# Aakash1312/Fluid-Simulation

Measured on AMD Instinct MI355X. Metric: simulated substeps/sec, higher is better.
Workload: dtype f64

## Files before the change

fluid-simulation_amd/_lib.py:

```python
import ctypes as C
import os

_HERE = os.path.dirname(os.path.abspath(__file__))
_SO = os.path.join(_HERE, "libfluid_hip.so")
if not os.path.exists(_SO):
    raise ImportError(
        f"{_SO} is missing: build it with `make -C {_HERE}` (hipcc --offload-arch=gfx950). "
        "This package has no CPU path.")
lib = C.CDLL(_SO)


class FluidError(RuntimeError):
    def __init__(self, code, msg):
        super().__init__(f"libfluid_hip error {code}: {msg}")
        self.code = code


class Params(C.Structure):
    _fields_ = [("n", C.c_int32), ("device", C.c_int32), ("dx", C.c_double), ("rho", C.c_double),
                ("gravity", C.c_double * 3), ("max_dt", C.c_double), ("outer_tol", C.c_double),
                ("update_frac", C.c_double), ("cg_tol", C.c_double), ("cg_max_iters", C.c_int32),
                ("max_outer_passes", C.c_int32), ("precision", C.c_int32), ("preconditioner", C.c_int32),
                ("flip_blend", C.c_double), ("solve_start", C.c_int32), ("mg_precision", C.c_int32),
                ("dist_solve", C.c_int32), ("pad_", C.c_int32)]
# ... 116 lines not shown
SYMBOLS = [
    ("fluid_default_params", C.c_int, [C.POINTER(Params)]),
    ("fluid_create", C.c_int, [C.POINTER(Params), C.POINTER(_P)]),
    ("fluid_destroy", C.c_int, [_P]),
    ("fluid_last_error", C.c_char_p, []),
    ("fluid_version", C.c_char_p, []),
    ("fluid_set_solid", C.c_int, [_P, _P]),
    ("fluid_upload_particles", C.c_int, [_P, C.c_int64, _P, _P]),
    ("fluid_download_particles", C.c_int, [_P, _P, _P]),
    ("fluid_num_particles", C.c_int64, [_P]),
    ("fluid_set_dt", C.c_int, [_P, C.c_double]),
    ("fluid_get_dt", C.c_int, [_P, C.POINTER(C.c_double)]),
    ("fluid_scene_water_cube_drop", C.c_int64, [C.c_int32, C.c_int32, C.c_uint64, _P]),
    ("fluid_scene_uniform_scatter", C.c_int64, [C.POINTER(C.c_int32), C.POINTER(C.c_int32), C.c_float, C.c_uint32, C.c_int32, _P]),
    ("fluid_step", C.c_int, [_P, C.POINTER(StepStats)]),
    ("fluid_p2g", C.c_int, [_P]),
    ("fluid_flags_index", C.c_int, [_P]),
    ("fluid_rhs_div", C.c_int, [_P, C.c_int]),
    ("fluid_solve", C.c_int, [_P]),
    ("fluid_vel_update", C.c_int, [_P]),
    ("fluid_pressure_pass", C.c_int, [_P, C.POINTER(C.c_double)]),
    ("fluid_flip_advect", C.c_int, [_P]),
    ("fluid_get_stats", C.c_int, [_P, C.POINTER(StepStats)]),
    ("fluid_download_field", C.c_int, [_P, C.c_int, _P, C.c_size_t]),
    ("fluid_upload_field", C.c_int, [_P, C.c_int, _P, C.c_size_t]),
    ("fluid_stencil_apply", C.c_int, [_P, C.c_int, C.c_int, C.POINTER(C.c_float)]),
    ("fluid_extrapolate", C.c_int, [_P, C.POINTER(C.c_int32)]),
    ("fluid_resample", C.c_int, [_P, C.c_int32, C.POINTER(C.c_int64)]),
    ("fluid_get_droplets", C.c_int, [_P, C.POINTER(C.c_int32), _P, C.c_int32]),
    ("fluid_add_particles", C.c_int, [_P, C.c_int64, _P, _P]),
    ("fluid_set_source", C.c_int, [_P, C.c_int32, C.POINTER(Source)]),
    ("fluid_set_sink", C.c_int, [_P, C.c_int32, C.POINTER(C.c_int32), C.POINTER(C.c_int32)]),
    ("fluid_get_source_stats", C.c_int, [_P, C.POINTER(C.c_int64), C.POINTER(C.c_int64), C.POINTER(C.c_int64), C.POINTER(C.c_int64)]),
    ("fluid_dist_set_source", C.c_int, [_P, C.c_int32, C.POINTER(Source)]),
    ("fluid_dist_set_sink", C.c_int, [_P, C.c_int32, C.POINTER(C.c_int32), C.POINTER(C.c_int32)]),
    ("fluid_dist_get_source_stats", C.c_int, [_P, C.POINTER(C.c_int64), C.POINTER(C.c_int64), C.POINTER(C.c_int64), C.POINTER(C.c_int64)]),
    ("fluid_dist_add_particles", C.c_int, [_P, C.c_int64, _P, _P, _P]),
    ("fluid_stencil_apply_hbm", C.c_int, [_P, C.c_int, C.c_int, C.c_int64, C.POINTER(C.c_int32), C.POINTER(C.c_float)]),
    ("fluid_profile_enable", C.c_int, [_P, C.c_int]),
    ("fluid_profile_read", C.c_int, [_P, C.c_int, C.POINTER(C.c_int64), C.POINTER(C.c_int64), C.POINTER(C.c_double), C.POINTER(C.c_double)]),
    ("fluid_profile_reset", C.c_int, [_P]),
    ("fluid_spline_eval", C.c_int, [C.c_int32, C.c_int32, C.c_int64, _P, _P]),
    ("fluid_dot_eval", C.c_int, [C.c_int32, C.c_int64, _P, _P, _P]),
    ("fluid_scan_eval", C.c_int, [C.c_int32, C.c_int32, C.c_int64, C.c_int32, C.c_int32, _P, _P, _P]),
    ("fluid_write_vdb", C.c_int, [C.c_char_p, C.c_int32, C.c_int32, C.POINTER(_P)]),
    ("fluid_write_vdb_ex", C.c_int, [C.c_char_p, C.c_int32, C.c_int32, C.POINTER(_P), C.c_int32]),
# ... 101 lines not shown
```

fluid-simulation_amd/csrc/common.h:

```cpp
#pragma once
#include <hip/hip_runtime.h>
#include <stdint.h>

namespace fl {

constexpr uint8_t F_SOLID = 1;
constexpr uint8_t F_FLUID = 2;
constexpr int F_CNT_SHIFT = 2;

struct Grid {
    int N;
    int lo;
    int hi;
    int nx, ny, nz;
    int ox, oy, oz;
    __host__ __device__ inline size_t idx(int ix, int iy, int iz) const
    {
        return ((size_t)ix * ny + (size_t)iy) * nz + (size_t)iz;
    }
    __host__ __device__ inline size_t cells() const { return (size_t)nx * ny * nz; }
    __host__ __device__ inline long sx() const { return (long)ny * nz; }
    __host__ __device__ inline int cx0() const { return lo + ox; }
    __host__ __device__ inline int cy0() const { return lo + oy; }
    __host__ __device__ inline int cz0() const { return lo + oz; }
// ... 41 lines not shown
};

struct PcgState {
    double bb;
    double thr;
    double rr;
    int done;
    int iters;
    int breakdown;
    int pad;
};

struct StepState {
    int bbox_min[3];
    int bbox_max[3];
    int num_active;
    int n_out;
    int max_cell;
    int n_drop;
    int n_tl_mg, n_tl_sq;
    int n_rows, n_l1_old;
    int n_tl_int, n_tl_bnd;
    int n_l1_gal, n_drop_fail;
    unsigned long long max_speed_bits;
    double dt;
    double err_num;
    double err_den;
};

constexpr size_t STATE_PS_OFF = 256;
constexpr int MAX_PARTIALS = 8192;

__device__ __forceinline__ double spline(double x)
{
    if (x < 0) x *= -1.0;
    if (x < 0.5) return 1.5 * (4.0 * x * x * x - 4.0 * x * x + 2.0 / 3.0);
    if (x < 1.0) return 1.5 * ((-8.0 * (x * x * x) / 6.0) + 4.0 * x * x - 4.0 * x + 4.0 / 3.0);
    return 0;
}

__device__ __forceinline__ double spline_at(double p, int c, int d)
{
    double x = p - (double)c;
    if (d == 1) return spline(x);
    if (x < 0) x *= -1.0;
    if (x < 1.0) return 1.5 * ((-8.0 * (x * x * x) / 6.0) + 4.0 * x * x - 4.0 * x + 4.0 / 3.0);
// ... 126 lines not shown
        return q;
    }
};
constexpr uint32_t PID_DEAD = 0xFFFFFFFFu;

void launch_bin_count(hipStream_t st, Grid g, long n, Particles p, int* key, int* slot, int* cell_count, int* part, StepState* ss);
void launch_bin_scatter(hipStream_t st, long n, const int* key, const int* slot, const int* cell_start, const uint32_t* pid, int* order,
                         uint32_t* spid);
void launch_bin_rank(hipStream_t st, long n_pos, long pos0, const int* key, const int* cell_start, const int* order, const uint32_t* spid,
                     int* order2);
void launch_reorder(hipStream_t st, long n, const int* order, Particles src, Particles dst, double* w = nullptr, long wstride = 0);
void launch_weights(hipStream_t st, long n, Particles p, double* w, long stride);
void launch_axpby_box(hipStream_t st, Grid g, Box box, double a, const double* x, double b, const double* y, double* out, const PcgState* gate = nullptr);
long p2g_max_items(Box box);
size_t p2g_part_doubles(Box box);
constexpr int P2G_PILED = 256;
void launch_p2g(hipStream_t st, Grid g, Box box, Particles p, const double* pw, long wstride, const int* cell_start, const uint8_t* flags,
                double* part, int* items, float* container, double* u, double* v, double* w, double* ub, double* vb, double* wb, int2* crowd_list = nullptr,
                Particles park = Particles{});
void launch_p2g_tiles(hipStream_t st, Grid g, Box box, Particles p, const double* pw, long wstride, const int* cell_start, const uint8_t* flags,
                      float* container, double* u, double* v, double* w, double* ub, double* vb, double* wb);
void launch_g2p_tiled(hipStream_t st, Grid g, Box pb, Particles p, const int* cell_start, const double* dcx, const double* dcy, const double* dcz,
                      const double* pcx, const double* pcy, const double* pcz, double blend, StepState* ss);
void launch_g2p(hipStream_t st, Grid g, long n, Particles p, const double* dcx, const double* dcy, const double* dcz, const double* pcx,
                const double* pcy, const double* pcz, double blend, StepState* ss);
void launch_advect(hipStream_t st, Grid g, long n, Particles p, const uint8_t* flags, double max_dt, double dx, StepState* ss);
void launch_advect_bin(hipStream_t st, Grid g, long n, Particles p, const uint8_t* flags, double max_dt, double dx, StepState* ss, int* key,
                       int* slot, int* cell_count, int* part);
void launch_pack_particles(hipStream_t st, long n, Particles p, double* pos_aos, double* vel_aos);
void launch_unpack_records(hipStream_t st, long n, const double* rec, Particles p, long off);
void launch_pack_records(hipStream_t st, long n, Particles p, long off, double* rec);
void launch_unpack_ids(hipStream_t st, long n, const double* pos, const double* vel, const uint32_t* ids, Particles p);
void launch_pack_ids(hipStream_t st, long n, Particles p, long off, double* pos, double* vel, uint32_t* ids);
void launch_unpack_particles(hipStream_t st, long n, const double* pos_aos, const double* vel_aos, Particles p);

struct OutWin {
    int ny, nz;
    int ox, oy, oz;
    int olo[3], ohi[3];
    int lo, off;
    int l0[3], nl[3];
    __host__ __device__ inline long leaves() const { return (long)nl[0] * nl[1] * nl[2]; }
};
void launch_out_mark(hipStream_t st, const float* f, const OutWin& w, int* flags);
void launch_out_pack(hipStream_t st, const float* f, const OutWin& w, const int* flags, const int* slot, float* values, int* origin);
struct SdfGeom {
// ... 211 lines not shown
```

fluid-simulation_amd/csrc/fluid_api.hip:

```cpp
#include "sim.h"
#include <algorithm>

using namespace fl;

static thread_local std::string g_err;
int fluid_fail(int code, const std::string& msg)
{
    g_err = msg;
    return code;
}
#define fail fluid_fail

Box fl::clip_dilate(const Box& b, int d, const Grid& g)
{
    Box r;
    r.x0 = b.x0 - d < 0 ? 0 : b.x0 - d;
    r.y0 = b.y0 - d < 0 ? 0 : b.y0 - d;
    r.z0 = b.z0 - d < 0 ? 0 : b.z0 - d;
    r.x1 = b.x1 + d > g.nx - 1 ? g.nx - 1 : b.x1 + d;
    r.y1 = b.y1 + d > g.ny - 1 ? g.ny - 1 : b.y1 + d;
    r.z1 = b.z1 + d > g.nz - 1 ? g.nz - 1 : b.z1 + d;
    return r;
}

// ... 184 lines not shown
    if (p->mg_precision != FLUID_MG_FP32 && p->mg_precision != FLUID_MG_FP64) return fail(FLUID_ERR_ARG, "bad mg_precision");
    if (p->dist_solve < FLUID_DIST_AUTO || p->dist_solve > FLUID_DIST_REPLICATED || p->pad_ != 0) return fail(FLUID_ERR_ARG, "bad dist_solve / pad_");
    int ndev = 0;
    if (hipGetDeviceCount(&ndev) != hipSuccess || ndev <= 0)
        return fail(FLUID_ERR_HIP, "no HIP device visible: libfluid_hip has no CPU path");
    if (p->device < 0 || p->device >= ndev) return fail(FLUID_ERR_ARG, "device ordinal out of range");
    HIPCHK(hipSetDevice(p->device));
    fluid_sim* s = new fluid_sim();
    s->prm = *p;
    s->g = g;
    s->ncell = g.cells();
    s->dt = p->max_dt;
    s->mg_fp32 = p->mg_precision == FLUID_MG_FP32;
    s->warm = p->solve_start == FLUID_START_WARM;
    if (const char* e = getenv("FLUID_MG_CSWEEPS")) s->mg_csweeps = atoi(e);
    if (const char* e = getenv("FLUID_TILE_LISTS")) s->lists_force = atoi(e) != 0;
    if (const char* e = getenv("FLUID_P2G_FORM")) s->p2g_force = !strcmp(e, "rows") ? 1 : (!strcmp(e, "tiles") ? 2 : (!strcmp(e, "crowd") ? 3 : 0));
    if (const char* e = getenv("FLUID_MG_GALERKIN")) s->gal_mode = atoi(e);
    if (const char* e = getenv("FLUID_DROPLETS")) s->drops_on = atoi(e) != 0;
    if (const char* e = getenv("FLUID_ROW_SWEEPS")) s->row_sweeps = atoi(e) != 0;
    if (const char* e = getenv("FLUID_DROPLETS_MIN")) s->drop_min = atoi(e);
    if (const char* e = getenv("FLUID_ADVECT_BIN")) s->advect_bin = atoi(e) != 0;
    if (const char* e = getenv("FLUID_SOLVE_TAIL")) s->solve_tail = atoi(e) != 0;
    *out = nullptr;
    auto bail = [&](int rc) { fluid_destroy(s); return rc; };
#define A(expr) do { hipError_t e_ = (expr); if (e_ != hipSuccess) return bail(fail(FLUID_ERR_HIP, std::string(#expr) + ": " + hipGetErrorString(e_))); } while (0)
    A(hipStreamCreateWithFlags(&s->st, hipStreamNonBlocking));
    const size_t n = s->ncell;
    A(dalloc(&s->solid, n)); A(dalloc(&s->flags, n));
    A(dalloc(&s->container, n)); A(dalloc(&s->rhs, n)); A(dalloc(&s->diver, n)); A(dalloc(&s->diver2, n));
    A(dalloc(&s->u, n)); A(dalloc(&s->v, n)); A(dalloc(&s->w, n));
    A(dalloc(&s->ub, n)); A(dalloc(&s->vb, n)); A(dalloc(&s->wb, n));
    A(dalloc(&s->dcx, n)); A(dalloc(&s->dcy, n)); A(dalloc(&s->dcz, n));
    A(dalloc(&s->pressure, n));
    if (s->warm) {
        A(dalloc(&s->p_guess, n)); A(dalloc(&s->p_guess2, n));
        if (hipMemset(s->p_guess, 0, n * sizeof(double)) != hipSuccess || hipMemset(s->p_guess2, 0, n * sizeof(double)) != hipSuccess) return bail(FLUID_ERR_HIP);
        if (const char* e = getenv("FLUID_EXTRAPOLATE")) s->extrapolate = atoi(e) != 0;
        if (s->extrapolate) { A(dalloc(&s->p_q, n)); if (hipMemset(s->p_q, 0, n * sizeof(double)) != hipSuccess) return bail(FLUID_ERR_HIP); }
    }
    A(dalloc(&s->indices, n));
    A(dalloc(&s->scan_sums, (n + 2) / 2048 + 16));
    A(dalloc(&s->ipart, (size_t)1024 * 8));
    const size_t se = solver_elem(s);
    s->lmax = lbox_max_cells(std::max(g.nx, std::max(g.ny, g.nz)));
    const size_t ln = s->lmax;
// ... 891 lines not shown
    if (error) *error = err;
    return FLUID_OK;
}

int fl::pic_fields(fluid_sim* s)
{
    if (s->prm.flip_blend >= 1.0 || s->pcx) return FLUID_OK;
    double** f[3] = {&s->pcx, &s->pcy, &s->pcz};
    for (double** q : f) {
        HIPCHK(hipMalloc((void**)q, s->ncell * sizeof(double)));
        HIPCHK(hipMemsetAsync(*q, 0, s->ncell * sizeof(double), s->st));
    }
    return FLUID_OK;
}

static int phase_flip_advect(fluid_sim* s)
{
    if (!s->have_p2g) return fail(FLUID_ERR_STATE, "flip_advect before p2g");
    HIPCHK(hipSetDevice(s->prm.device));
    int rcp = pic_fields(s);
    if (rcp) return rcp;
    if (!box_empty(s->Rb)) launch_flip_delta(s->st, s->g, s->Rb, s->u, s->v, s->w, s->ub, s->vb, s->wb, s->dcx, s->dcy, s->dcz, s->pcx, s->pcy, s->pcz);
    int tok = prof_begin(s, FLUID_PROF_G2P, (double)s->np);
    if (s->sorted && s->p_off == 0 && (double)s->np >= 4.0 * (double)s->Pb.cells()) {
        launch_g2p_tiled(s->st, s->g, s->Pb, s->pa, s->cell_start, s->dcx, s->dcy, s->dcz, s->pcx, s->pcy, s->pcz, s->prm.flip_blend, s->ss);
        if (!box_empty(s->Pb)) s->stats.paths |= FLUID_PATH_G2P_TILES;
        if (s->n_out > 0)
            launch_g2p(s->st, s->g, s->n_out, s->pa.shifted(s->np - s->n_out), s->dcx, s->dcy, s->dcz, s->pcx, s->pcy, s->pcz, s->prm.flip_blend, s->ss);
    } else {
        launch_g2p(s->st, s->g, s->np, s->pa.shifted(s->p_off), s->dcx, s->dcy, s->dcz, s->pcx, s->pcy, s->pcz, s->prm.flip_blend, s->ss);
    }
    prof_end(s, FLUID_PROF_G2P, tok);
    const bool bin = s->advect_bin && !s->dist && s->np > 0 && s->sorted && s->sort_hint && !box_empty(s->Pb);
    s->binned = false;
    if (bin) {
        const Grid g = s->g;
        s->bin_x0 = std::max(0, s->Pb.x0 - 3);
        s->bin_x1 = std::min(g.nx - 1, s->Pb.x1 + 3);
        const long n2 = g.sx(), c0 = (long)s->bin_x0 * n2, c1 = (long)(s->bin_x1 + 1) * n2;
        HIPCHK(hipMemsetAsync(s->cell_count + c0, 0, (c1 - c0) * sizeof(int), s->st));
        HIPCHK(hipMemsetAsync(s->cell_count + s->ncell, 0, 4 * sizeof(int), s->st));
        launch_advect_bin(s->st, g, s->np, s->pa.shifted(s->p_off), s->flags, s->prm.max_dt, s->prm.dx, s->ss, s->key, s->slot, s->cell_count, s->ipart);
    } else {
        launch_advect(s->st, s->g, s->np, s->pa.shifted(s->p_off), s->flags, s->prm.max_dt, s->prm.dx, s->ss);
    }
    HIPCHK(hipGetLastError());
    int rc = read_ss(s);
    if (rc) return rc;
    if (bin) {
        const StepState& h = *s->h_ss;
        for (int a = 0; a < 3; ++a) s->bin_min[a] = h.bbox_min[a], s->bin_max[a] = h.bbox_max[a];
        s->bin_n_out = h.n_out;
        s->bin_max_cell = h.max_cell;
        s->binned = true;
    }
    s->dt = s->h_ss->dt;
    double ms;
    memcpy(&ms, &s->h_ss->max_speed_bits, sizeof(double));
    s->stats.max_speed = ms;
    s->stats.dt_out = s->dt;
    s->sorted = false;
    s->have_p2g = false;
    s->vel_ok = true;
    return FLUID_OK;
}

extern "C" {

#define PHASE_GUARD(s)                                                                                        \
    if (!(s)) return fail(FLUID_ERR_ARG, "null handle");                                                      \
    if ((s)->dist) return fail(FLUID_ERR_STATE, "per-phase entry points are single-GPU only; a decomposed run steps with fluid_step")
int fluid_p2g(fluid_sim_t* s) { PHASE_GUARD(s); return phase_p2g(s); }
int fluid_flags_index(fluid_sim_t* s) { PHASE_GUARD(s); return phase_flags(s); }
int fluid_rhs_div(fluid_sim_t* s, int which) { PHASE_GUARD(s); return phase_rhs_div(s, which, nullptr); }
int fluid_solve(fluid_sim_t* s) { PHASE_GUARD(s); return phase_solve(s, false); }
int fluid_vel_update(fluid_sim_t* s) { PHASE_GUARD(s); return phase_vel_update(s, nullptr); }
int fluid_pressure_pass(fluid_sim_t* s, double* error) { PHASE_GUARD(s); return phase_pressure_pass(s, error); }
int fluid_flip_advect(fluid_sim_t* s) { PHASE_GUARD(s); return phase_flip_advect(s); }
// ... 58 lines not shown
        std::sort(o, o + m);
        for (int q = m; q < 64; ++q) o[q] = -1;
    }
    return FLUID_OK;
}

int fluid_resample(fluid_sim_t* s, int32_t per_cell, int64_t* n_parked)
{
    PHASE_GUARD(s);
    if (per_cell < 0) return fail(FLUID_ERR_ARG, "per_cell must be >= 0");
    if (s->np == 0) { if (n_parked) *n_parked = 0; return FLUID_OK; }
    HIPCHK(hipSetDevice(s->prm.device));
    int rc = phase_sort(s);
    if (rc) return rc;
    HIPCHK(hipMemsetAsync(s->d_small, 0, sizeof(int), s->st));
    launch_resample(s->st, s->g, s->np - s->n_out, s->pa, s->cell_start, per_cell, s->g.hi - 10, (double)(s->g.hi + 40), s->d_small);
    HIPCHK(hipGetLastError());
    HIPCHK(hipMemcpyAsync(s->h_small, s->d_small, sizeof(int), hipMemcpyDeviceToHost, s->st));
    HIPCHK(hipStreamSynchronize(s->st));
    if (n_parked) *n_parked = s->h_small[0];
    s->sorted = s->have_p2g = s->have_flags = false;
    s->sort_hint = false;
    s->binned = false;
    return FLUID_OK;
}

int fluid_get_stats(fluid_sim_t* s, fluid_step_stats_t* st)
{
    if (!s || !st) return fail(FLUID_ERR_ARG, "null argument");
    *st = s->stats;
    return FLUID_OK;
}


int fluid_step(fluid_sim_t* s, fluid_step_stats_t* stats)
{
    if (!s) return fail(FLUID_ERR_ARG, "null handle");
    int rc;
    if ((rc = output_auto_check(s))) return rc;
    if (s->dist) return dist_step(s, stats);
    if ((rc = phase_p2g(s))) return rc;
    if ((rc = phase_flags(s))) return rc;
    double error = NAN;
    do {
        if ((rc = phase_pressure_pass(s, &error))) return rc;
        if (s->prm.max_outer_passes > 0 && s->stats.outer_passes >= s->prm.max_outer_passes) break;
// ... 247 lines not shown
```

fluid-simulation_amd/csrc/kernels_grid.hip:

```cpp
#include "common.h"

namespace fl {

constexpr int SCAN_T = 256;
constexpr int SCAN_E = 8;
constexpr int SCAN_CHUNK = SCAN_T * SCAN_E;

template <int MODE>
__device__ __forceinline__ int scan_load(const void* in, long i)
{
    if (MODE == 0) return ((const int*)in)[i];
    return (((const uint8_t*)in)[i] & F_FLUID) ? 1 : 0;
}

template <int MODE, bool VEC>
__device__ __forceinline__ void scan_load8(const void* in, long base, long n, int v[SCAN_E])
{
    if (VEC && base >= 0 && base + SCAN_E <= n) {
        if (MODE == 0) {
            const int4 a = *(const int4*)((const int*)in + base), b = *(const int4*)((const int*)in + base + 4);
            v[0] = a.x; v[1] = a.y; v[2] = a.z; v[3] = a.w;
            v[4] = b.x; v[5] = b.y; v[6] = b.z; v[7] = b.w;
        } else {
            const uint2 w = *(const uint2*)((const uint8_t*)in + base);
// ... 475 lines not shown
    double num = 0, den = 0;
    for (int i = threadIdx.x; i < nb; i += 256) { num += part[2 * i]; den += part[2 * i + 1]; }
    num = block_sum<double, 4>(num, sm);
    den = block_sum<double, 4>(den, sm);
    if (threadIdx.x == 0) { ss->err_num = num; ss->err_den = den; }
}

void launch_err_norm(hipStream_t st, Grid g, Box box, const uint8_t* flags, const float* b, const float* b2, double* part, StepState* ss, const PcgState* gate)
{
    long nb = (box.cells() + 255) / 256;
    if (nb > 1024) nb = 1024;
    if (nb < 1) nb = 1;
    hipLaunchKernelGGL(k_err_partial, dim3((unsigned)nb), dim3(256), 0, st, g, box, flags, b, b2, part, gate);
    hipLaunchKernelGGL(k_err_final, dim3(1), dim3(256), 0, st, (const double*)part, (int)nb, ss, gate);
}

__global__ void k_zero_step_state(StepState* ss, int N)
{
    ss->bbox_min[0] = ss->bbox_min[1] = ss->bbox_min[2] = N;
    ss->bbox_max[0] = ss->bbox_max[1] = ss->bbox_max[2] = -1;
    ss->num_active = 0;
    ss->n_out = 0;
    ss->n_drop_fail = 0;
    ss->max_speed_bits = 0ull;
    ss->err_num = 0;
    ss->err_den = 0;
}
void launch_zero_step_state(hipStream_t st, StepState* ss, int N)
{
    hipLaunchKernelGGL(k_zero_step_state, dim3(1), dim3(1), 0, st, ss, N);
}

__global__ void k_sort_tail(const int* __restrict__ cell_count, int* __restrict__ cell_start, long c1, long ncell)
{
    const int t = cell_start[c1];
    cell_start[ncell] = t;
    cell_start[ncell + 1] = t + cell_count[ncell];
    cell_start[ncell + 2] = t + cell_count[ncell] + cell_count[ncell + 1];
}
void launch_sort_tail(hipStream_t st, const int* cell_count, int* cell_start, long c1, long ncell)
{
    hipLaunchKernelGGL(k_sort_tail, dim3(1), dim3(1), 0, st, cell_count, cell_start, c1, ncell);
}

__global__ __launch_bounds__(256) void k_zero_fields(ZeroList z, Grid g, Box box)
{
// ... 179 lines not shown
```

fluid-simulation_amd/csrc/kernels_particles.hip:

```cpp
#include "common.h"

namespace fl {

struct BinAcc {
    int mn[3] = {0x7fffffff, 0x7fffffff, 0x7fffffff}, mx[3] = {-1, -1, -1};
    int nout = 0, cmax = 0;
};
__device__ __forceinline__ void bin_one(const Grid& g, long ncell, long i, double px, double py, double pz, bool dead, int* __restrict__ key,
                                        int* __restrict__ slot, int* __restrict__ cell_count, BinAcc& acc)
{
    int bx = (int)round(px) - g.cx0(), by = (int)round(py) - g.cy0(), bz = (int)round(pz) - g.cz0();
    bool in = bx >= 0 && bx < g.nx && by >= 0 && by < g.ny && bz >= 0 && bz < g.nz;
    int k = in ? (int)g.idx(bx, by, bz) : (int)ncell;
    if (dead) { k = (int)ncell + 1; in = false; }
    key[i] = k;
    {
        const int lane = threadIdx.x & 63;
        const int kp = __shfl_up(k, 1, 64);
        const bool head = lane == 0 || kp != k;
        const unsigned long long hm = __ballot(head);
        const unsigned long long below = hm & ((2ull << lane) - 1ull);
        const int start = 63 - __clzll((long long)below);
        const unsigned long long above = (lane == 63) ? 0ull : (hm >> (lane + 1)) << (lane + 1);
        const unsigned long long act = __ballot(true);
// ... 828 lines not shown
                vz += d2 / weight;
                if (PIC) {
                    vx = blend * vx + (1.0 - blend) * (q0 / weight);
                    vy = blend * vy + (1.0 - blend) * (q1 / weight);
                    vz = blend * vz + (1.0 - blend) * (q2 / weight);
                }
                p.vx[i] = vx; p.vy[i] = vy; p.vz[i] = vz;
            }
            double l = sqrt(vx * vx + vy * vy + vz * vz);
            if (!(l == l)) l = 0;
            len = l > len ? l : len;
        }
    }
    len = wave_max(len);
    if ((tid & 63) == 0) sm[tid >> 6] = len;
    __syncthreads();
    if (tid == 0) {
        double m = sm[0];
        for (int k = 1; k < 4; ++k) m = sm[k] > m ? sm[k] : m;
        if (m > 0) atomicMax(&ss->max_speed_bits, (unsigned long long)__double_as_longlong(m));
    }
}

__device__ __forceinline__ bool is_solid(const Grid& g, const uint8_t* flags, int x, int y, int z)
{
    if (x < g.cx0() || x > g.cx1() || y < g.cy0() || y > g.cy1() || z < g.cz0() || z > g.cz1()) return false;
    return flags[g.idx(x - g.cx0(), y - g.cy0(), z - g.cz0())] & F_SOLID;
}

__device__ __forceinline__ double advect_timestep(double max_dt, double dx, const StepState* ss)
{
    const double maxSpeed = __longlong_as_double((long long)ss->max_speed_bits);
    if (maxSpeed != 0) return max_dt < dx / maxSpeed ? max_dt : dx / maxSpeed;
    return max_dt;
}
__device__ __forceinline__ void advect_one(const Grid& g, const Particles& p, const uint8_t* __restrict__ flags, double timestep, long i, double& P0,
                                           double& P1, double& P2)
{
    const double e = 0;
    P0 = p.px[i], P1 = p.py[i], P2 = p.pz[i];
    double V0 = p.vx[i], V1 = p.vy[i], V2 = p.vz[i];
    const double q0 = P0 + timestep * V0, q1 = P1 + timestep * V1, q2 = P2 + timestep * V2;
    if (is_solid(g, flags, (int)round(q0), (int)round(q1), (int)round(q2))) {
        const double vx = V0 * timestep, vy = V1 * timestep, vz = V2 * timestep;
        if (is_solid(g, flags, (int)round(P0 + vx), (int)P1, (int)P2)) V0 *= -1.0 * e;
        if (is_solid(g, flags, (int)P0, (int)round(P1 + vy), (int)P2)) V1 *= -1.0 * e;
// ... 169 lines not shown
        hipLaunchKernelGGL(k_p2g_crowd_list, dim3(nblk((long)sb.nx() * sb.ny() * ((sb.nz() + 3) / 4))), dim3(256), 0, st, g, sb, cell_start, crowd_list, items + 1);
        hipLaunchKernelGGL(k_p2g_crowd_sum, dim3(2048), dim3(64 * PC_WAVES), 0, st, p, pw, wstride, crowd_list, items + 1, park);
        if (vec) hipLaunchKernelGGL((k_p2g_rows<true, true>), dim3(nt), dim3(P2G_THREADS), 0, st, g, box, p, pw, wstride, cell_start, part, cells, zt, items, park, colflag, ntz);
        else hipLaunchKernelGGL((k_p2g_rows<false, true>), dim3(nt), dim3(P2G_THREADS), 0, st, g, box, p, pw, wstride, cell_start, part, cells, zt, items, park, colflag, ntz);
    } else if (vec) hipLaunchKernelGGL((k_p2g_rows<true, false>), dim3(nt), dim3(P2G_THREADS), 0, st, g, box, p, pw, wstride, cell_start, part, cells, zt, items, park, colflag, ntz);
    else hipLaunchKernelGGL((k_p2g_rows<false, false>), dim3(nt), dim3(P2G_THREADS), 0, st, g, box, p, pw, wstride, cell_start, part, cells, zt, items, park, colflag, ntz);
    hipLaunchKernelGGL(k_p2g_combine, dim3(nblk(cells)), dim3(256), 0, st, g, box, part, cells, flags, container, u, v, w, ub, vb, wb, items, colflag, zt, ntz);
}
void launch_p2g_tiles(hipStream_t st, Grid g, Box box, Particles p, const double* pw, long wstride, const int* cell_start, const uint8_t* flags,
                      float* container, double* u, double* v, double* w, double* ub, double* vb, double* wb)
{
    const int ntz = (box.nz() + P2G_ZT - 1) / P2G_ZT, zt = (box.nz() + ntz - 1) / ntz;
    const unsigned nt = (unsigned)(((box.nx() + P2GT_T - 1) / P2GT_T) * ((box.ny() + P2GT_T - 1) / P2GT_T) * ntz);
    hipLaunchKernelGGL(k_p2g_tiles, dim3(nt), dim3(P2GT_THREADS), 0, st, g, box, p, pw, wstride, cell_start, flags, container, u, v, w, ub, vb, wb, zt);
}
void launch_g2p_tiled(hipStream_t st, Grid g, Box pb, Particles p, const int* cell_start, const double* dcx, const double* dcy, const double* dcz,
                      const double* pcx, const double* pcy, const double* pcz, double blend, StepState* ss)
{
    if (pb.cells() <= 0) return;
    const unsigned nt = (unsigned)(((pb.nx() + G2P_TX - 1) / G2P_TX) * ((pb.ny() + G2P_TY - 1) / G2P_TY) * ((pb.nz() + G2P_TZ - 1) / G2P_TZ));
    if (pcx) hipLaunchKernelGGL(k_g2p_tiled<true>, dim3(nt), dim3(256), 0, st, g, pb, p, cell_start, dcx, dcy, dcz, pcx, pcy, pcz, blend, ss);
    else hipLaunchKernelGGL(k_g2p_tiled<false>, dim3(nt), dim3(256), 0, st, g, pb, p, cell_start, dcx, dcy, dcz, pcx, pcy, pcz, blend, ss);
}
void launch_g2p(hipStream_t st, Grid g, long n, Particles p, const double* dcx, const double* dcy, const double* dcz, const double* pcx,
                const double* pcy, const double* pcz, double blend, StepState* ss)
{
    if (n > 0) hipLaunchKernelGGL(k_g2p, dim3(nblk(n)), dim3(256), 0, st, g, n, p, dcx, dcy, dcz, pcx, pcy, pcz, blend, ss);
}
void launch_advect(hipStream_t st, Grid g, long n, Particles p, const uint8_t* flags, double max_dt, double dx, StepState* ss)
{
    if (n > 0) hipLaunchKernelGGL(k_advect, dim3(nblk(n)), dim3(256), 0, st, g, n, p, flags, max_dt, dx, ss);
    hipLaunchKernelGGL(k_publish_dt, dim3(1), dim3(1), 0, st, max_dt, dx, ss, (const int*)nullptr, 0);
}
void launch_advect_bin(hipStream_t st, Grid g, long n, Particles p, const uint8_t* flags, double max_dt, double dx, StepState* ss, int* key,
                       int* slot, int* cell_count, int* part)
{
    unsigned nb = nblk(n);
    if (nb > 1024) nb = 1024;
    hipLaunchKernelGGL(k_advect_bin, dim3(nb), dim3(256), 0, st, g, n, p, flags, max_dt, dx, ss, key, slot, cell_count, part);
    hipLaunchKernelGGL(k_publish_dt, dim3(1), dim3(256), 0, st, max_dt, dx, ss, (const int*)part, (int)nb);
}
void launch_unpack_records(hipStream_t st, long n, const double* rec, Particles p, long off)
{
    if (n > 0) hipLaunchKernelGGL(k_unpack_records, dim3(nblk(n)), dim3(256), 0, st, n, rec, p, off);
}
void launch_pack_records(hipStream_t st, long n, Particles p, long off, double* rec)
// ... 22 lines not shown
```

fluid-simulation_amd/csrc/sim.h:

```cpp
#pragma once
#include "common.h"
#include "../../include/fluid_hip.h"

#include <cmath>
#include <cstdio>
#include <cstdlib>
#include <cstring>
#include <string>
#include <utility>
#include <vector>

int fluid_fail(int code, const std::string& msg);
#define HIPCHK(expr)                                                                                              \
    do {                                                                                                          \
        hipError_t e_ = (expr);                                                                                   \
        if (e_ != hipSuccess)                                                                                     \
            return fluid_fail(FLUID_ERR_HIP, std::string(#expr) + ": " + hipGetErrorString(e_) + " @" + std::to_string(__LINE__)); \
    } while (0)
#include "snap_ring.h"

using namespace fl;

struct ProfClass {
    long launches = 0, sampled = 0;
// ... 76 lines not shown
    int* drop_n = nullptr;
    int* drop_cells = nullptr;
    int n_drop = 0;
    int drop_last = -1;
    int drop_min = 4000;
    int drop_skipped = 0;
    bool lists_hint = false;
    bool lists_on = false;
    int lists_force = -1;
    int p2g_force = 0;
    long p2g_ref_cells = 0;
    long last_num_active = 0;
    StepState* ss = nullptr;
    StepState* h_ss = nullptr;
    Box Pb{0, 0, 0, -1, -1, -1}, Rb{0, 0, 0, -1, -1, -1}, Sb{0, 0, 0, -1, -1, -1};
    Box dirty{0, 0, 0, -1, -1, -1};
    int flag_x0 = 0, flag_x1 = -1;
    bool flags_valid = false;
    bool sorted = false, have_p2g = false, have_flags = false;
    long n_out = 0;
    bool sort_hint = false;
    bool advect_bin = true;
    bool binned = false;
    int bin_x0 = 0, bin_x1 = -1;
    int bin_min[3] = {0, 0, 0}, bin_max[3] = {-1, -1, -1}, bin_n_out = 0, bin_max_cell = 0;
    bool solve_tail = true;
    bool tail_ran = false;
    double dt = 0.1;
    fluid_step_stats_t stats{};
    static constexpr int MG_MAXL = 8;
    int mg_nl = 0, mg_tail = 0;
    long mg_last_iters_k[3] = {0, 0, 0};
    int pass_class() const { return stats.outer_passes < 2 ? stats.outer_passes : 2; }
    int mg_csweeps = 3;
    MLevel mgl[MG_MAXL];
    uint8_t *mg_typ[MG_MAXL] = {}, *mg_cnt[MG_MAXL] = {};
    int gal_mode = 1;
    int gal_it[2] = {-1, -1};
    int gal_since_probe = 0;
    bool gal_eligible = false;
    bool gal = false;
    int gal_lc = 0;
    double gal_dt = 0;
    double gal_wc = 1.8;
    int gal_sweeps = 3;
    char* gal_slab = nullptr;
// ... 150 lines not shown
```

fluid-simulation_amd/sim.py:

```python
import ctypes as C
import numpy as np

from ._lib import lib, check, FluidError, Params, StepStats, FIELD, Source, LeafGridC, SdfParams, SdfGridC, SdfFilter, SdfTrack, MeshC, SdfAttrC, MeshAttrC, SdfAttrPartC, MeshExC, MESH, Camera, Shade, ImageC, RENDER

_FIELD_DTYPE = {
    FIELD.CONTAINER: (np.float32, 1), FIELD.WEIGHTS: (np.float32, 1), FIELD.OUTPUT: (np.float32, 1),
    FIELD.VEL: (np.float64, 3), FIELD.VEL_BEFORE: (np.float64, 3), FIELD.INDICES: (np.int32, 1),
    FIELD.RHS: (np.float32, 1), FIELD.DIVER: (np.float32, 1), FIELD.DIVER2: (np.float32, 1),
    FIELD.PRESSURE: (np.float64, 1), FIELD.SOLID: (np.uint8, 1), FIELD.FLAGS: (np.uint8, 1),
}


def grid_bounds(n):
    lo = -(n // 2)
    return lo, lo + n - 1


_VDB_COMPRESSION = {"zip": 3, "active_mask": 2}


def write_vdb(path, grids, compression="zip"):
    import ctypes as C
    if isinstance(grids, np.ndarray) and grids.ndim == 3:
        grids = [grids]
# ... 593 lines not shown

    def rhs_div(self, which=0):
        check(lib.fluid_rhs_div(self._h, which))

    def solve(self):
        check(lib.fluid_solve(self._h))

    def vel_update(self):
        check(lib.fluid_vel_update(self._h))

    def pressure_pass(self):
        e = C.c_double()
        check(lib.fluid_pressure_pass(self._h, C.byref(e)))
        return e.value

    def flip_advect(self):
        check(lib.fluid_flip_advect(self._h))

    def stats(self):
        st = StepStats()
        check(lib.fluid_get_stats(self._h, C.byref(st)))
        return st.as_dict()

    def _solver_dtype(self):
        return np.float64 if self.precision == "fp64" else np.float32

    def field(self, fid):
        if fid in (FIELD.SEARCH, FIELD.Q):
            dt, comps = self._solver_dtype(), 1
        else:
            dt, comps = _FIELD_DTYPE[fid]
        n = self.n
        arr = np.empty((comps, n, n, n) if comps > 1 else (n, n, n), dtype=dt)
        check(lib.fluid_download_field(self._h, fid, arr.ctypes.data_as(C.c_void_p), arr.nbytes))
        return arr

    def upload_field(self, fid, arr):
        if fid in (FIELD.SEARCH, FIELD.Q):
            dt = self._solver_dtype()
        else:
            dt = _FIELD_DTYPE[fid][0]
        a = np.ascontiguousarray(arr, dtype=dt)
        check(lib.fluid_upload_field(self._h, fid, a.ctypes.data_as(C.c_void_p), a.nbytes))

    def output_snapshot(self):
        check(lib.fluid_output_snapshot(self._h))
# ... 170 lines not shown
```

include/fluid_hip.h:

```cpp
#ifndef FLUID_HIP_H
#define FLUID_HIP_H

#include <stddef.h>
#include <stdint.h>

#ifdef __cplusplus
extern "C" {
#endif

typedef struct fluid_sim fluid_sim_t;

#define FLUID_OK 0
#define FLUID_ERR_ARG 1
#define FLUID_ERR_HIP 2
#define FLUID_ERR_STATE 3
#define FLUID_ERR_SOLVER 4
#define FLUID_ERR_PEER 5

#define FLUID_FIELD_CONTAINER 0
#define FLUID_FIELD_WEIGHTS 1
#define FLUID_FIELD_VEL 2
#define FLUID_FIELD_VEL_BEFORE 3
#define FLUID_FIELD_INDICES 4
#define FLUID_FIELD_RHS 5
// ... 47 lines not shown
    double dt_in;
    double dt_out;
    double error;
    double max_speed;
    double relres;
    int64_t num_active;
    int32_t outer_passes;
    int32_t cg_iters;
    int32_t cg_iters_last;
    int32_t box_lo[3];
    int32_t box_hi[3];
    int32_t paths;
} fluid_step_stats_t;
#define FLUID_PATH_P2G_TILES 1
#define FLUID_PATH_P2G_CROWD 16
#define FLUID_PATH_TILE_LISTS 2
#define FLUID_PATH_DIST_DECOMPOSED 4
#define FLUID_PATH_DIST_REPLICATED 8
#define FLUID_PATH_DIST_REBALANCED 32
#define FLUID_PATH_MG_GALERKIN 128
#define FLUID_PATH_DROPLETS 64
#define FLUID_PATH_DROPLETS_SHORT 256
#define FLUID_PATH_G2P_TILES 1024

int fluid_default_params(fluid_params_t* p);
int fluid_create(const fluid_params_t* p, fluid_sim_t** out);
int fluid_destroy(fluid_sim_t* s);
const char* fluid_last_error(void);
const char* fluid_version(void);

int fluid_set_solid(fluid_sim_t* s, const uint8_t* solid);
int fluid_upload_particles(fluid_sim_t* s, int64_t n, const double* pos, const double* vel);
int fluid_download_particles(fluid_sim_t* s, double* pos, double* vel);
int64_t fluid_num_particles(fluid_sim_t* s);
int fluid_set_dt(fluid_sim_t* s, double dt);
int fluid_get_dt(fluid_sim_t* s, double* dt);
int64_t fluid_scene_water_cube_drop(int32_t n, int32_t ppc, uint64_t seed, double* pos);
int64_t fluid_scene_uniform_scatter(const int32_t lo[3], const int32_t hi[3], float points_per_volume, uint32_t seed,
                                    int32_t boundary, double* pos);

int fluid_step(fluid_sim_t* s, fluid_step_stats_t* stats);

int fluid_p2g(fluid_sim_t* s);
int fluid_flags_index(fluid_sim_t* s);
int fluid_rhs_div(fluid_sim_t* s, int which);
int fluid_solve(fluid_sim_t* s);
int fluid_vel_update(fluid_sim_t* s);
int fluid_pressure_pass(fluid_sim_t* s, double* error);
int fluid_flip_advect(fluid_sim_t* s);
int fluid_get_stats(fluid_sim_t* s, fluid_step_stats_t* stats);

int fluid_download_field(fluid_sim_t* s, int field, void* dst, size_t bytes);
int fluid_upload_field(fluid_sim_t* s, int field, const void* src, size_t bytes);

int fluid_extrapolate(fluid_sim_t* s, int32_t* n_layers);
int fluid_resample(fluid_sim_t* s, int32_t per_cell, int64_t* n_parked);

#define FLUID_MAX_SOURCES 8
#define FLUID_MAX_SINKS 8
#define FLUID_SOURCE_ADD 0
#define FLUID_SOURCE_FILL 1
#define FLUID_SOURCE_VEL_FIXED 0
#define FLUID_SOURCE_VEL_GRID 1
#define FLUID_PATH_SOURCES 512
typedef struct fluid_source {
    int32_t lo[3], hi[3];
    int32_t per_cell;
    int32_t mode;
    int32_t every;
    int32_t vel_mode;
    double vel[3];
    uint64_t seed;
} fluid_source_t;
// ... 234 lines not shown
```

Baseline: 157.9.

## Add wave-cooperative row-window G2P kernel for sorted sparse particle sets

Adds a G2P kernel in which each wavefront loads up to two shared 3x3x16 grid windows into LDS, taken from the cell of the first particle and the first outlier. Particles that fall inside a window interpolate from LDS, and the rest gather directly from global memory. By default (mode 2) it replaces the generic per-particle gather when particles are sorted but not dense enough for the tiled path. The aim is to cut redundant global reads of the grid velocity fields. In exchange it adds LDS pressure, block-wide syncs and extra counter atomics, plus a debug API for the LDS-hit and own-gather counts.

```diff
diff --git a/fluid-simulation_amd/_lib.py b/fluid-simulation_amd/_lib.py
--- a/fluid-simulation_amd/_lib.py
+++ b/fluid-simulation_amd/_lib.py
@@ -162,6 +162,7 @@
     ("fluid_pressure_pass", C.c_int, [_P, C.POINTER(C.c_double)]),
     ("fluid_flip_advect", C.c_int, [_P]),
     ("fluid_get_stats", C.c_int, [_P, C.POINTER(StepStats)]),
+    ("fluid_g2p_counts", C.c_int, [_P, C.POINTER(C.c_int64)]),
     ("fluid_download_field", C.c_int, [_P, C.c_int, _P, C.c_size_t]),
     ("fluid_upload_field", C.c_int, [_P, C.c_int, _P, C.c_size_t]),
     ("fluid_stencil_apply", C.c_int, [_P, C.c_int, C.c_int, C.POINTER(C.c_float)]),
diff --git a/fluid-simulation_amd/csrc/common.h b/fluid-simulation_amd/csrc/common.h
--- a/fluid-simulation_amd/csrc/common.h
+++ b/fluid-simulation_amd/csrc/common.h
@@ -87,6 +87,7 @@
     int n_rows, n_l1_old;
     int n_tl_int, n_tl_bnd;
     int n_l1_gal, n_drop_fail;
+    int g2p_lds, g2p_own;
     unsigned long long max_speed_bits;
     double dt;
     double err_num;
@@ -259,6 +260,8 @@
                       float* container, double* u, double* v, double* w, double* ub, double* vb, double* wb);
 void launch_g2p_tiled(hipStream_t st, Grid g, Box pb, Particles p, const int* cell_start, const double* dcx, const double* dcy, const double* dcz,
                       const double* pcx, const double* pcy, const double* pcz, double blend, StepState* ss);
+void launch_g2p_rows(hipStream_t st, Grid g, long n, const int* n_on, Particles p, const double* dcx, const double* dcy, const double* dcz,
+                     const double* pcx, const double* pcy, const double* pcz, double blend, StepState* ss);
 void launch_g2p(hipStream_t st, Grid g, long n, Particles p, const double* dcx, const double* dcy, const double* dcz, const double* pcx,
                 const double* pcy, const double* pcz, double blend, StepState* ss);
 void launch_advect(hipStream_t st, Grid g, long n, Particles p, const uint8_t* flags, double max_dt, double dx, StepState* ss);
diff --git a/fluid-simulation_amd/csrc/fluid_api.hip b/fluid-simulation_amd/csrc/fluid_api.hip
--- a/fluid-simulation_amd/csrc/fluid_api.hip
+++ b/fluid-simulation_amd/csrc/fluid_api.hip
@@ -230,6 +230,7 @@
     if (const char* e = getenv("FLUID_DROPLETS_MIN")) s->drop_min = atoi(e);
     if (const char* e = getenv("FLUID_ADVECT_BIN")) s->advect_bin = atoi(e) != 0;
     if (const char* e = getenv("FLUID_SOLVE_TAIL")) s->solve_tail = atoi(e) != 0;
+    if (const char* e = getenv("FLUID_G2P")) s->g2p_mode = !strcmp(e, "tiles") ? 0 : (!strcmp(e, "rows") ? 1 : 2);
     *out = nullptr;
     auto bail = [&](int rc) { fluid_destroy(s); return rc; };
 #define A(expr) do { hipError_t e_ = (expr); if (e_ != hipSuccess) return bail(fail(FLUID_ERR_HIP, std::string(#expr) + ": " + hipGetErrorString(e_))); } while (0)
@@ -1167,7 +1168,17 @@
     if (rcp) return rcp;
     if (!box_empty(s->Rb)) launch_flip_delta(s->st, s->g, s->Rb, s->u, s->v, s->w, s->ub, s->vb, s->wb, s->dcx, s->dcy, s->dcz, s->pcx, s->pcy, s->pcz);
     int tok = prof_begin(s, FLUID_PROF_G2P, (double)s->np);
-    if (s->sorted && s->p_off == 0 && (double)s->np >= 4.0 * (double)s->Pb.cells()) {
+    const bool sorted1 = s->sorted && s->p_off == 0;
+    const bool dense = sorted1 && (double)s->np >= 4.0 * (double)s->Pb.cells();
+    const long n_on = s->np - s->n_out;
+    const bool rows = sorted1 && n_on > 0 && (s->g2p_mode == 1 || (s->g2p_mode == 2 && !dense));
+    if (rows) {
+        launch_g2p_rows(s->st, s->g, n_on, s->cell_start + s->ncell, s->pa, s->dcx, s->dcy, s->dcz, s->pcx, s->pcy, s->pcz, s->prm.flip_blend, s->ss);
+        if (s->g2p_mode == 1) s->stats.paths |= FLUID_PATH_G2P_ROWS;
+        if (dense && !box_empty(s->Pb)) s->stats.paths |= FLUID_PATH_G2P_TILES;
+        if (s->n_out > 0)
+            launch_g2p(s->st, s->g, s->n_out, s->pa.shifted(s->np - s->n_out), s->dcx, s->dcy, s->dcz, s->pcx, s->pcy, s->pcz, s->prm.flip_blend, s->ss);
+    } else if (dense) {
         launch_g2p_tiled(s->st, s->g, s->Pb, s->pa, s->cell_start, s->dcx, s->dcy, s->dcz, s->pcx, s->pcy, s->pcz, s->prm.flip_blend, s->ss);
         if (!box_empty(s->Pb)) s->stats.paths |= FLUID_PATH_G2P_TILES;
         if (s->n_out > 0)
@@ -1199,6 +1210,8 @@
         s->bin_max_cell = h.max_cell;
         s->binned = true;
     }
+    s->g2p_counts[0] = rows ? s->h_ss->g2p_lds : 0;
+    s->g2p_counts[1] = rows ? s->h_ss->g2p_own : 0;
     s->dt = s->h_ss->dt;
     double ms;
     memcpy(&ms, &s->h_ss->max_speed_bits, sizeof(double));
@@ -1303,6 +1316,13 @@
     s->sorted = s->have_p2g = s->have_flags = false;
     s->sort_hint = false;
     s->binned = false;
+    return FLUID_OK;
+}
+
+int fluid_g2p_counts(fluid_sim_t* s, int64_t out[2])
+{
+    if (!s || !out) return fail(FLUID_ERR_ARG, "null argument");
+    out[0] = s->g2p_counts[0], out[1] = s->g2p_counts[1];
     return FLUID_OK;
 }
 
diff --git a/fluid-simulation_amd/csrc/kernels_grid.hip b/fluid-simulation_amd/csrc/kernels_grid.hip
--- a/fluid-simulation_amd/csrc/kernels_grid.hip
+++ b/fluid-simulation_amd/csrc/kernels_grid.hip
@@ -521,6 +521,7 @@
     ss->num_active = 0;
     ss->n_out = 0;
     ss->n_drop_fail = 0;
+    ss->g2p_lds = ss->g2p_own = 0;
     ss->max_speed_bits = 0ull;
     ss->err_num = 0;
     ss->err_den = 0;
diff --git a/fluid-simulation_amd/csrc/kernels_particles.hip b/fluid-simulation_amd/csrc/kernels_particles.hip
--- a/fluid-simulation_amd/csrc/kernels_particles.hip
+++ b/fluid-simulation_amd/csrc/kernels_particles.hip
@@ -874,6 +874,159 @@
     }
 }
 
+constexpr int G2P_RZ = 14, G2P_RW = G2P_RZ + 2, G2P_RSLOT = 9 * G2P_RW;
+template <bool PIC>
+__global__ __launch_bounds__(256, PIC ? 2 : 4) void k_g2p_rows(Grid g, const int* __restrict__ n_on_p, Particles p,
+                                                               const double* __restrict__ dcx, const double* __restrict__ dcy,
+                                                               const double* __restrict__ dcz, const double* __restrict__ pcx,
+                                                               const double* __restrict__ pcy, const double* __restrict__ pcz, double blend,
+                                                               StepState* ss)
+{
+    constexpr int NF = PIC ? 6 : 3;
+    __shared__ double sf[NF][4][2 * G2P_RSLOT];
+    __shared__ double sm[4];
+    __shared__ int sc[4][2];
+    const int tid = threadIdx.x, lane = tid & 63, wv = tid >> 6;
+    const long n_on = *n_on_p, nrun = (n_on + 255) / 256;
+    double len = 0;
+    int n_lds = 0, n_own = 0;
+    for (long u = blockIdx.x; u < nrun; u += gridDim.x) {
+        const long i = u * 256 + tid;
+        const bool act = i < n_on;
+        double cx = 0, cy = 0, cz = 0, vx = 0, vy = 0, vz = 0;
+        if (act) cx = p.px[i], cy = p.py[i], cz = p.pz[i], vx = p.vx[i], vy = p.vy[i], vz = p.vz[i];
+        const int fcx = (int)round(cx), fcy = (int)round(cy), fcz = (int)round(cz);
+        const int bx = fcx - g.cx0(), by = fcy - g.cy0(), bz = fcz - g.cz0();
+        const int xA = __builtin_amdgcn_readfirstlane(bx), yA = __builtin_amdgcn_readfirstlane(by), zA = __builtin_amdgcn_readfirstlane(bz);
+        const bool inA = act && bx == xA && by == yA && (unsigned)(bz - zA) < (unsigned)G2P_RZ;
+        const unsigned long long rest = __ballot(act && !inA);
+        const int lB = rest ? __ffsll((long long)rest) - 1 : 0;
+        const int xB = __builtin_amdgcn_readfirstlane(__shfl(bx, lB, 64)), yB = __builtin_amdgcn_readfirstlane(__shfl(by, lB, 64)),
+                  zB = __builtin_amdgcn_readfirstlane(__shfl(bz, lB, 64));
+        const bool inB = act && !inA && bx == xB && by == yB && (unsigned)(bz - zB) < (unsigned)G2P_RZ;
+        const bool own = act && !inA && !inB;
+        const int nwin = __builtin_amdgcn_readfirstlane(act) ? (rest ? 2 : 1) : 0;
+        for (int s = 0; s < nwin; ++s) {
+            const int X = s ? xB : xA, Y = s ? yB : yA, Z = s ? zB : zA;
+            const int zz = lane & 15, gz = Z - 1 + zz;
+            double val[3][NF];
+            bool in[3];
+#pragma unroll
+            for (int k = 0; k < 3; ++k) {
+                const int r = min(4 * k + (lane >> 4), 8);
+                const int gx = X - 1 + r / 3, gy = Y - 1 + r % 3;
+                in[k] = gx >= 0 && gx < g.nx && gy >= 0 && gy < g.ny && gz >= 0 && gz < g.nz;
+                const size_t c = g.idx(min(max(gx, 0), g.nx - 1), min(max(gy, 0), g.ny - 1), min(max(gz, 0), g.nz - 1));
+                val[k][0] = dcx[c], val[k][1] = dcy[c], val[k][2] = dcz[c];
+                if (PIC) val[k][PIC ? 3 : 0] = pcx[c], val[k][PIC ? 4 : 0] = pcy[c], val[k][PIC ? 5 : 0] = pcz[c];
+            }
+#pragma unroll
+            for (int k = 0; k < 3; ++k) {
+                const int r = 4 * k + (lane >> 4);
+                if (r < 9) {
+                    const int t = s * G2P_RSLOT + r * G2P_RW + zz;
+#pragma unroll
+                    for (int f = 0; f < NF; ++f) sf[f][wv][t] = in[k] ? val[k][f] : 0.0;
+                }
+            }
+        }
+        __syncthreads();
+        if (act) {
+            const int wlo = g.lo + 2, whi = g.hi - 2;
+            double wx[3], wy[3], wz[3];
+#pragma unroll
+            for (int d = 0; d < 3; ++d) {
+                const int ax = fcx - 1 + d, ay = fcy - 1 + d, az = fcz - 1 + d;
+                wx[d] = (ax >= wlo && ax <= whi) ? spline_at(cx, ax, d) : 0.0;
+                wy[d] = (ay >= wlo && ay <= whi) ? spline_at(cy, ay, d) : 0.0;
+                wz[d] = (az >= wlo && az <= whi) ? spline_at(cz, az, d) : 0.0;
+            }
+            double weight = 0, d0 = 0, d1 = 0, d2 = 0, q0 = 0, q1 = 0, q2 = 0;
+            if (!own) {
+                const int lb = inA ? bz - zA : G2P_RSLOT + (bz - zB);
+#pragma unroll
+                for (int xi = 0; xi < 3; ++xi)
+#pragma unroll
+                    for (int yi = 0; yi < 3; ++yi)
+#pragma unroll
+                        for (int zi = 0; zi < 3; ++zi) {
+                            const int c = lb + (xi * 3 + yi) * G2P_RW + zi;
+                            const double cw = wx[xi] * wy[yi] * wz[zi];
+                            weight += cw;
+                            d0 += sf[0][wv][c] * cw;
+                            d1 += sf[1][wv][c] * cw;
+                            d2 += sf[2][wv][c] * cw;
+                            if (PIC) {
+                                q0 += sf[PIC ? 3 : 0][wv][c] * cw;
+                                q1 += sf[PIC ? 4 : 0][wv][c] * cw;
+                                q2 += sf[PIC ? 5 : 0][wv][c] * cw;
+                            }
+                        }
+            } else {
+                const int sxs = (int)g.sx();
+                int oy[3], oz[3];
+#pragma unroll
+                for (int d = 0; d < 3; ++d) {
+                    oy[d] = min(max(by - 1 + d, 0), g.ny - 1) * g.nz;
+                    oz[d] = min(max(bz - 1 + d, 0), g.nz - 1);
+                }
+#pragma unroll 1
+                for (int xi = 0; xi < 3; ++xi) {
+                    const double wxi = xi == 0 ? wx[0] : xi == 1 ? wx[1] : wx[2];
+                    const int ox = min(max(bx - 1 + xi, 0), g.nx - 1) * sxs;
+                    double f[9][NF];
+#pragma unroll
+                    for (int k = 0; k < 9; ++k) {
+                        const int c = ox + oy[k / 3] + oz[k % 3];
+                        f[k][0] = dcx[c], f[k][1] = dcy[c], f[k][2] = dcz[c];
+                        if (PIC) f[k][PIC ? 3 : 0] = pcx[c], f[k][PIC ? 4 : 0] = pcy[c], f[k][PIC ? 5 : 0] = pcz[c];
+                    }
+#pragma unroll
+                    for (int k = 0; k < 9; ++k) {
+                        const double cw = wxi * wy[k / 3] * wz[k % 3];
+                        weight += cw;
+                        d0 += f[k][0] * cw;
+                        d1 += f[k][1] * cw;
+                        d2 += f[k][2] * cw;
+                        if (PIC) {
+                            q0 += f[k][PIC ? 3 : 0] * cw;
+                            q1 += f[k][PIC ? 4 : 0] * cw;
+                            q2 += f[k][PIC ? 5 : 0] * cw;
+                        }
+                    }
+                }
+            }
+            if (weight != 0) {
+                vx += d0 / weight;
+                vy += d1 / weight;
+                vz += d2 / weight;
+                if (PIC) {
+                    vx = blend * vx + (1.0 - blend) * (q0 / weight);
+                    vy = blend * vy + (1.0 - blend) * (q1 / weight);
+                    vz = blend * vz + (1.0 - blend) * (q2 / weight);
+                }
+                p.vx[i] = vx; p.vy[i] = vy; p.vz[i] = vz;
+            }
+            double l = sqrt(vx * vx + vy * vy + vz * vz);
+            if (!(l == l)) l = 0;
+            len = l > len ? l : len;
+        }
+        n_lds += __popcll(__ballot(act && !own)), n_own += __popcll(__ballot(own));
+        __syncthreads();
+    }
+    len = wave_max(len);
+    if (lane == 0) sm[wv] = len, sc[wv][0] = n_lds, sc[wv][1] = n_own;
+    __syncthreads();
+    if (tid == 0) {
+        double m = sm[0];
+        for (int k = 1; k < 4; ++k) m = sm[k] > m ? sm[k] : m;
+        if (m > 0) atomicMax(&ss->max_speed_bits, (unsigned long long)__double_as_longlong(m));
+        const int a = sc[0][0] + sc[1][0] + sc[2][0] + sc[3][0], b = sc[0][1] + sc[1][1] + sc[2][1] + sc[3][1];
+        if (a) atomicAdd(&ss->g2p_lds, a);
+        if (b) atomicAdd(&ss->g2p_own, b);
+    }
+}
+
 __device__ __forceinline__ bool is_solid(const Grid& g, const uint8_t* flags, int x, int y, int z)
 {
     if (x < g.cx0() || x > g.cx1() || y < g.cy0() || y > g.cy1() || z < g.cz0() || z > g.cz1()) return false;
@@ -1089,6 +1242,15 @@
     if (pcx) hipLaunchKernelGGL(k_g2p_tiled<true>, dim3(nt), dim3(256), 0, st, g, pb, p, cell_start, dcx, dcy, dcz, pcx, pcy, pcz, blend, ss);
     else hipLaunchKernelGGL(k_g2p_tiled<false>, dim3(nt), dim3(256), 0, st, g, pb, p, cell_start, dcx, dcy, dcz, pcx, pcy, pcz, blend, ss);
 }
+void launch_g2p_rows(hipStream_t st, Grid g, long n, const int* n_on, Particles p, const double* dcx, const double* dcy, const double* dcz,
+                     const double* pcx, const double* pcy, const double* pcz, double blend, StepState* ss)
+{
+    if (n <= 0) return;
+    const long nrun = nblk(n), slots = 256 * (pcx ? 2 : 4), per = (nrun + slots - 1) / slots;
+    const unsigned nb = (unsigned)((nrun + per - 1) / per);
+    if (pcx) hipLaunchKernelGGL(k_g2p_rows<true>, dim3(nb), dim3(256), 0, st, g, n_on, p, dcx, dcy, dcz, pcx, pcy, pcz, blend, ss);
+    else hipLaunchKernelGGL(k_g2p_rows<false>, dim3(nb), dim3(256), 0, st, g, n_on, p, dcx, dcy, dcz, pcx, pcy, pcz, blend, ss);
+}
 void launch_g2p(hipStream_t st, Grid g, long n, Particles p, const double* dcx, const double* dcy, const double* dcz, const double* pcx,
                 const double* pcy, const double* pcz, double blend, StepState* ss)
 {
diff --git a/fluid-simulation_amd/csrc/sim.h b/fluid-simulation_amd/csrc/sim.h
--- a/fluid-simulation_amd/csrc/sim.h
+++ b/fluid-simulation_amd/csrc/sim.h
@@ -122,6 +122,8 @@
     bool sort_hint = false;
     bool advect_bin = true;
     bool binned = false;
+    int g2p_mode = 2;
+    int64_t g2p_counts[2] = {0, 0};
     int bin_x0 = 0, bin_x1 = -1;
     int bin_min[3] = {0, 0, 0}, bin_max[3] = {-1, -1, -1}, bin_n_out = 0, bin_max_cell = 0;
     bool solve_tail = true;
diff --git a/fluid-simulation_amd/sim.py b/fluid-simulation_amd/sim.py
--- a/fluid-simulation_amd/sim.py
+++ b/fluid-simulation_amd/sim.py
@@ -639,6 +639,11 @@
         check(lib.fluid_get_stats(self._h, C.byref(st)))
         return st.as_dict()
 
+    def g2p_counts(self):
+        out = (C.c_int64 * 2)()
+        check(lib.fluid_g2p_counts(self._h, out))
+        return int(out[0]), int(out[1])
+
     def _solver_dtype(self):
         return np.float64 if self.precision == "fp64" else np.float32
 
diff --git a/include/fluid_hip.h b/include/fluid_hip.h
--- a/include/fluid_hip.h
+++ b/include/fluid_hip.h
@@ -93,6 +93,7 @@
 #define FLUID_PATH_DROPLETS 64
 #define FLUID_PATH_DROPLETS_SHORT 256
 #define FLUID_PATH_G2P_TILES 1024
+#define FLUID_PATH_G2P_ROWS 2048
 
 int fluid_default_params(fluid_params_t* p);
 int fluid_create(const fluid_params_t* p, fluid_sim_t** out);
@@ -120,6 +121,7 @@
 int fluid_pressure_pass(fluid_sim_t* s, double* error);
 int fluid_flip_advect(fluid_sim_t* s);
 int fluid_get_stats(fluid_sim_t* s, fluid_step_stats_t* stats);
+int fluid_g2p_counts(fluid_sim_t* s, int64_t out[2]);
 
 int fluid_download_field(fluid_sim_t* s, int field, void* dst, size_t bytes);
 int fluid_upload_field(fluid_sim_t* s, int field, const void* src, size_t bytes);
```

Measured after the change: 159.7 (median of 6 runs). 1.1% higher.
